# ruffle-rs/h263-rs

Hardware: NVIDIA B200
Metric: decoded_rgba_megapixels_per_s (higher is better)
Workload: dtype f32+u8

## Files before the change

### h263_rs_b200/csrc/context.cu

```cuda
#include <cuda_runtime.h>

#include <algorithm>
#include <chrono>
#include <cstdio>
#include <cstdlib>
#include <cstring>
#include <mutex>
#include <new>
#include <vector>

#include "device_math.cuh"
#include "kernels.cuh"

using namespace h263dev;

namespace h263fe {
int parse_step_deferred(h263cu_parser* const* parsers, const uint8_t* const* packets, const size_t* lens,
                        const uint32_t* stream_ids, uint32_t n, int threads, h263cu_pic* pics, h263cu_mb* mbs, uint32_t mb_cap,
                        h263cu_event* events, uint32_t ev_cap, uint32_t* n_pics_out, uint32_t* n_mbs_out, uint32_t* n_units_out,
                        int* per_pic_err, int32_t* pic_of_input, uint32_t max_w, uint32_t max_h);
void parse_step_finish(h263cu_parser* const* parsers, uint32_t n, bool accept);
}

extern "C" const uint8_t h263cu_quant_to_strength[32] = H263_QUANT_TO_STRENGTH;

namespace {

#define CU_TRY(expr)                      \
    do {                                  \
        cudaError_t _e = (expr);          \
        if (_e != cudaSuccess) return map_cuda_error(_e); \
    } while (0)

int map_cuda_error(cudaError_t e) {
    switch (e) {
        case cudaErrorNoDevice:
        case cudaErrorInsufficientDriver:
        case cudaErrorInvalidDevice: return H263CU_ERR_NO_DEVICE;
        case cudaErrorMemoryAllocation: return H263CU_ERR_OUT_OF_MEMORY;
        default: return H263CU_ERR_CUDA;
    }
}

inline size_t round_up(size_t v, size_t a) { return (v + a - 1) / a * a; }

struct StreamState {
    bool has_pic = false;
    uint8_t cur_slot = 0;
    int8_t rgba_slot = -1;
    uint16_t w = 0, h = 0;
    uint8_t pic_type = 0, pquant = 0;
    uint16_t tr = 0;
    uint32_t stamp = 0;
    uint32_t seen = 0;
    bool has_ref = false;
    uint8_t ref_slot = 0;
    uint16_t ref_w = 0, ref_h = 0;
    bool padded = false;
};

inline int next_slot(const StreamState& st) { return st.has_ref ? (st.ref_slot ^ 1) : (st.has_pic ? (st.cur_slot ^ 1) : 0); }

inline void advance_stream(StreamState& st, const h263cu_pic& p, bool want_rgba, int rgba_ring, bool tiled) {
    const int slot = next_slot(st);
    st.cur_slot = (uint8_t)slot;
    st.has_pic = true;
    st.w = p.width, st.h = p.height;
    st.pic_type = p.pic_type, st.pquant = p.pquant, st.tr = p.temporal_reference;
    st.rgba_slot = want_rgba ? (int8_t)rgba_ring : (int8_t)-1;
    if (!(p.flags & H263CU_PICFLAG_DISPOSABLE)) {
        st.has_ref = true;
        st.ref_slot = (uint8_t)slot;
        st.ref_w = p.width, st.ref_h = p.height;
        st.padded = tiled;
    }
}

}

struct h263cu_step {
    std::vector<h263cu_pic> pics;
    h263cu_mb* d_mbs = nullptr;
    h263cu_event* d_events = nullptr;
    uint32_t n_mbs = 0, n_units = 0;
    size_t mb_cap = 0, ev_cap = 0;
    uint32_t max_w = 0, max_h = 0;
};

struct h263cu_ctx {
    int device = 0;
    uint32_t max_streams = 0, max_w = 0, max_h = 0;
    uint32_t mbw = 0, mbh = 0;
    uint32_t pitch_y = 0, pitch_c = 0, rgba_pitch = 0;
    size_t y_slot = 0, c_slot = 0, rgba_slot = 0;
    uint8_t *y_pool = nullptr, *c_pool = nullptr, *rgba_pool = nullptr;
    CUtensorMap rgba_map;
    std::vector<StreamState> streams;
    uint32_t stamp = 0, decode_epoch = 0;
    uint32_t rgba_parity = 0;

    cudaStream_t s_main = nullptr, s_h2d = nullptr, s_d2h = nullptr;
    cudaStream_t s_pics = nullptr;
    static constexpr int PIC_RING = 4;
    PicDev* h_pics[PIC_RING] = {};
    PicDev* d_pics[PIC_RING] = {};
    cudaEvent_t pics_done[PIC_RING] = {};
    cudaEvent_t pics_up[PIC_RING] = {};
    size_t pics_cap = 0;
    int pic_ring_pos = 0;
    h263cu_step ring[2];
    cudaEvent_t ring_h2d_done[2] = {}, ring_run_done[2] = {};
    int ring_pos = 0;
    struct Staging {
        h263cu_pic* pics = nullptr;
        h263cu_mb* mbs = nullptr;
        h263cu_event* events = nullptr;
        size_t pic_cap = 0, mb_cap = 0, ev_cap = 0;
    } staging[2];
    std::vector<int32_t> pic_of_input;
    std::vector<uint64_t> rgba_offsets;
    cudaEvent_t rgba_written[2] = {}, rgba_read[2] = {};
    cudaEvent_t t0 = nullptr, t1 = nullptr;
    uint64_t launches = 0, tiled_launches = 0;
    bool profiling = false;
    std::vector<cudaEvent_t> prof_free;
    struct ProfSpan {
        cudaEvent_t a, b;
        int kind;
    };
    std::vector<ProfSpan> prof_spans;
    ChecksumJob* d_jobs = nullptr;
    unsigned long long* d_sums = nullptr;
    size_t jobs_cap = 0;

    int force_kernel = 0;
    double host_parse_s = 0.0, host_other_s = 0.0;
    uint64_t host_calls = 0;
    uint8_t* plane(int p, uint32_t stream, int slot) const {
        const size_t idx = (size_t)stream * 2 + (size_t)slot;
        if (p == 0) return y_pool + idx * y_slot + (size_t)PAD_Y_ROWS * pitch_y + PAD_Y_COLS;
        return c_pool + idx * c_slot + (size_t)PAD_C_ROWS * pitch_c + PAD_C_COLS + (p == 2 ? 1 : 0);
    }
    uint8_t* rgba(uint32_t stream, int slot) const { return rgba_pool + ((size_t)slot * max_streams + stream) * rgba_slot; }
};

namespace {

int ensure_pic_ring(h263cu_ctx* c, size_t n) {
    if (n <= c->pics_cap) return 0;
    CU_TRY(cudaStreamSynchronize(c->s_main));
    size_t cap = std::max<size_t>(n, 256);
    for (int i = 0; i < h263cu_ctx::PIC_RING; i++) {
        if (c->h_pics[i]) cudaFreeHost(c->h_pics[i]);
        if (c->d_pics[i]) cudaFree(c->d_pics[i]);
        c->h_pics[i] = nullptr, c->d_pics[i] = nullptr;
        CU_TRY(cudaHostAlloc((void**)&c->h_pics[i], cap * sizeof(PicDev), cudaHostAllocDefault));
        CU_TRY(cudaMalloc((void**)&c->d_pics[i], cap * sizeof(PicDev)));
    }
    c->pics_cap = cap;
    return 0;
}

int step_reserve(h263cu_step* s, size_t n_mbs, size_t n_units) {
    if (n_mbs > s->mb_cap) {
        if (s->d_mbs) cudaFree(s->d_mbs);
        s->d_mbs = nullptr;
        size_t cap = n_mbs + n_mbs / 8 + 64;
        CU_TRY(cudaMalloc((void**)&s->d_mbs, cap * sizeof(h263cu_mb)));
        s->mb_cap = cap;
    }
    if (n_units + 8 > s->ev_cap) {
        if (s->d_events) cudaFree(s->d_events);
        s->d_events = nullptr;
        size_t cap = n_units + n_units / 8 + 64;
        CU_TRY(cudaMalloc((void**)&s->d_events, cap * sizeof(h263cu_event)));
        s->ev_cap = cap;
    }
    return 0;
}

int prof_take(h263cu_ctx* c, cudaEvent_t* a, cudaEvent_t* b) {
    for (cudaEvent_t* e : {a, b}) {
        if (!c->prof_free.empty()) {
            *e = c->prof_free.back();
            c->prof_free.pop_back();
        } else {
            CU_TRY(cudaEventCreate(e));
        }
    }
    return 0;
// ... 3 lines not shown
    c->prof_spans.push_back({a, b, kind});
}

PicDev make_picdev(const h263cu_ctx* c, const h263cu_pic& p, const StreamState& st, bool want_rgba, int rgba_ring) {
    const int ref_slot = st.ref_slot, new_slot = next_slot(st);
    PicDev d;
    std::memset(&d, 0, sizeof(d));
    for (int k = 0; k < 3; k++) {
        d.cur[k] = c->plane(k, p.stream, new_slot);
        d.ref[k] = st.has_ref ? c->plane(k, p.stream, ref_slot) : nullptr;
    }
    d.rgba = want_rgba ? c->rgba(p.stream, rgba_ring) : nullptr;
    d.cur_y4 = (uint32_t)((d.cur[0] - c->y_pool) >> 2);
    d.cur_c4 = (uint32_t)((d.cur[1] - c->c_pool) >> 2);
    d.ref_y4 = st.has_ref ? (uint32_t)((d.ref[0] - c->y_pool) >> 2) : 0u;
    d.ref_c4 = st.has_ref ? (uint32_t)((d.ref[1] - c->c_pool) >> 2) : 0u;
    d.rgba_row0 = want_rgba ? (uint32_t)((size_t)(d.rgba - c->rgba_pool) / c->rgba_pitch) : 0u;
    d.first_event = p.first_event;
    d.rgba_pitch = c->rgba_pitch;
    d.w = p.width, d.h = p.height;
    d.cw = (uint16_t)((p.width + 1) / 2), d.ch = (uint16_t)((p.height + 1) / 2);
    d.pitch_y = (uint16_t)c->pitch_y, d.pitch_c = (uint16_t)c->pitch_c;
    d.strength = h263cu_quant_to_strength[p.pquant & 31];
    d.flags = p.flags;
    return d;
}

int run_step(h263cu_ctx* c, h263cu_step* s, uint32_t out_flags, bool lean = false) {
    const uint32_t n = (uint32_t)s->pics.size();
    if (n == 0) return 0;
    if (n > 65535) return H263CU_ERR_CAPACITY;
    const bool want_rgba = (out_flags & H263CU_OUT_RGBA) != 0;
    const bool want_deblock = want_rgba && (out_flags & H263CU_OUT_DEBLOCK) != 0;
    const uint32_t stamp = ++c->stamp;
    uint32_t max_w = 0, max_h = 0;
    bool tiled = true, aligned16 = true, wide_mv = false;
    for (uint32_t i = 0; i < n; i++) {
        const h263cu_pic& p = s->pics[i];
        if (p.stream >= c->max_streams) return H263CU_ERR_CAPACITY;
        if (p.width == 0 || p.height == 0 || p.width > c->max_w || p.height > c->max_h) return H263CU_ERR_CAPACITY;
        if ((uint32_t)p.mb_w * 16 < p.width || (uint32_t)p.mb_h * 16 < p.height ||
            (uint32_t)p.mb_w > c->mbw || (uint32_t)p.mb_h > c->mbh)
            return H263CU_ERR_BAD_ARGUMENT;
        if ((uint64_t)p.first_mb + p.n_mbs > s->n_mbs || (uint64_t)p.first_event + p.n_event_units > s->n_units ||
            p.n_mbs != (uint32_t)p.mb_w * p.mb_h)
            return H263CU_ERR_BAD_ARGUMENT;
        StreamState& st = c->streams[p.stream];
        if (st.stamp == stamp) return H263CU_ERR_BAD_ARGUMENT;
        st.stamp = stamp;
        if (p.flags & H263CU_PICFLAG_HAS_INTER) {
            if (!st.has_ref) return H263CU_ERR_UNCODED_IFRAME_BLOCKS;
            if (st.ref_w != p.width || st.ref_h != p.height) return H263CU_ERR_REFERENCE_WOULD_ABORT;
        }
        max_w = std::max<uint32_t>(max_w, p.width);
        max_h = std::max<uint32_t>(max_h, p.height);
        if ((p.width | p.height) & 15) aligned16 = false;
        if ((p.flags & H263CU_PICFLAG_HAS_INTER) && !(p.flags & H263CU_PICFLAG_MV_IN_RANGE)) wide_mv = true;
        if ((p.flags & H263CU_PICFLAG_HAS_INTER) && !st.padded) tiled = false;
    }
    if (c->force_kernel == 1) tiled = false;
    int e = ensure_pic_ring(c, n);
    if (e) return e;
    const int slot = c->pic_ring_pos;
    CU_TRY(cudaEventSynchronize(c->pics_done[slot]));
    const int rgba_ring = (int)(c->rgba_parity & 1u);
    PicDev* hp = c->h_pics[slot];
    for (uint32_t i = 0; i < n; i++) {
        const h263cu_pic& p = s->pics[i];
        const PicDev d = make_picdev(c, p, c->streams[p.stream], want_rgba, rgba_ring);
        hp[i] = d;
    }
    cudaEvent_t pa = nullptr, pb = nullptr, qa = nullptr, qb = nullptr;
    if (c->profiling) {
        if ((e = prof_take(c, &pa, &pb))) return e;
        if (want_deblock && (e = prof_take(c, &qa, &qb))) {
            c->prof_free.push_back(pa), c->prof_free.push_back(pb);
            return e;
        }
    }
    if (lean) {
        CU_TRY(cudaMemcpyAsync(c->d_pics[slot], hp, n * sizeof(PicDev), cudaMemcpyHostToDevice, c->s_main));
    } else {
        CU_TRY(cudaMemcpyAsync(c->d_pics[slot], hp, n * sizeof(PicDev), cudaMemcpyHostToDevice, c->s_pics));
        CU_TRY(cudaEventRecord(c->pics_up[slot], c->s_pics));
        CU_TRY(cudaStreamWaitEvent(c->s_main, c->pics_up[slot], 0));
    }
    if (want_rgba) {
        CU_TRY(cudaStreamWaitEvent(c->s_main, c->rgba_read[rgba_ring], 0));
    }
    if (pa) cudaEventRecord(pa, c->s_main);
    const Pools pools{c->y_pool, c->c_pool, c->rgba_pool, c->pitch_y, c->pitch_c, c->rgba_pitch};
    launch_recon(c->d_pics[slot], s->d_mbs, s->d_events, s->n_mbs, want_rgba && !want_deblock, tiled ? (aligned16 ? 1 : 2) : 0, wide_mv, pools,
                 &c->rgba_map, c->s_main);
    if (pa) prof_end(c, pa, pb, 0);
    if (want_deblock) {
        if (qa) cudaEventRecord(qa, c->s_main);
        if (aligned16 && c->force_kernel != 1)
            launch_deblock_rgba_tile(c->d_pics[slot], n, max_w, max_h, c->s_main);
        else
            launch_deblock_rgba(c->d_pics[slot], n, max_w, max_h, c->s_main);
        if (qa) prof_end(c, qa, qb, 1);
    }
    CU_TRY(cudaGetLastError());
    c->pic_ring_pos = (c->pic_ring_pos + 1) % h263cu_ctx::PIC_RING;
    c->launches += want_deblock ? 2 : 1;
    if (tiled) c->tiled_launches++;
    for (uint32_t i = 0; i < n; i++) advance_stream(c->streams[s->pics[i].stream], s->pics[i], want_rgba, rgba_ring, tiled);
    CU_TRY(cudaEventRecord(c->pics_done[slot], c->s_main));
    if (want_rgba) {
        if (!lean) CU_TRY(cudaEventRecord(c->rgba_written[rgba_ring], c->s_main));
        c->rgba_parity++;
    }
    return 0;
}

int validate_side_info(std::vector<h263cu_pic>& pics, const h263cu_mb* mbs, uint32_t n_mbs, uint32_t n_units) {
    for (size_t i = 0; i < pics.size(); i++) {
        h263cu_pic& p = pics[i];
        if ((uint64_t)p.first_mb + p.n_mbs > n_mbs || (uint64_t)p.first_event + p.n_event_units > n_units ||
            p.n_mbs != (uint32_t)p.mb_w * p.mb_h || p.mb_w == 0)
            return H263CU_ERR_BAD_ARGUMENT;
        bool any_inter = false, in_range = true;
        const h263cu_mb* m = mbs + p.first_mb;
        for (uint32_t k = 0; k < p.n_mbs; k++, m++) {
            if (m->pic != i || (uint32_t)m->mby * p.mb_w + m->mbx != k || m->mbx >= p.mb_w) return H263CU_ERR_BAD_ARGUMENT;
            uint32_t ev = 0;
            for (int b = 0; b < 6; b++) ev += m->nev[b];
            if (m->flags & H263CU_MB_WIDE) ev *= 2;
            if ((uint64_t)m->ev_off + ev > p.n_event_units) return H263CU_ERR_BAD_ARGUMENT;
            if (m->flags & H263CU_MB_INTER) {
                any_inter = true;
                for (int b = 0; b < 4; b++)
                    in_range &= m->u.mv[b][0] >= -32 && m->u.mv[b][0] <= 31 && m->u.mv[b][1] >= -32 && m->u.mv[b][1] <= 31;
            }
        }
        if (any_inter) p.flags |= H263CU_PICFLAG_HAS_INTER;
        if (!in_range) p.flags &= (uint8_t)~H263CU_PICFLAG_MV_IN_RANGE;
    }
    return 0;
}

int upload_into(h263cu_ctx* c, h263cu_step* s, const h263cu_pic* pics, uint32_t n_pics, const h263cu_mb* mbs,
                uint32_t n_mbs, const h263cu_event* events, uint32_t n_units, cudaStream_t stream, bool trusted) {
    int e = step_reserve(s, n_mbs, n_units);
    if (e) return e;
    try {
        s->pics.assign(pics, pics + n_pics);
    } catch (const std::bad_alloc&) {
        return H263CU_ERR_OUT_OF_MEMORY;
    }
    s->n_mbs = n_mbs, s->n_units = n_units;
    if (!trusted && (e = validate_side_info(s->pics, mbs, n_mbs, n_units))) {
        s->pics.clear();
        return e;
    }
    if (n_mbs) CU_TRY(cudaMemcpyAsync(s->d_mbs, mbs, (size_t)n_mbs * sizeof(h263cu_mb), cudaMemcpyHostToDevice, stream));
    if (n_units)
        CU_TRY(cudaMemcpyAsync(s->d_events, events, (size_t)n_units * sizeof(h263cu_event), cudaMemcpyHostToDevice, stream));
    (void)c;
    return 0;
}

template <typename T>
int grow_pinned(T** p, size_t* cap, size_t need) {
    if (need <= *cap) return 0;
    if (*p) cudaFreeHost(*p);
    *p = nullptr, *cap = 0;
    const size_t n = need + need / 4 + 64;
    CU_TRY(cudaHostAlloc((void**)p, n * sizeof(T), cudaHostAllocDefault));
    *cap = n;
    return 0;
// ... 17 lines not shown
        return H263CU_ERR_CUDA;
    return 0;
}
void free_step_buffers(h263cu_step* s) {
    if (s->d_mbs) cudaFree(s->d_mbs);
    if (s->d_events) cudaFree(s->d_events);
    s->d_mbs = nullptr, s->d_events = nullptr;
    s->mb_cap = s->ev_cap = 0;
}

}

extern "C" {

int h263cu_device_count(void) {
    int n = 0;
    if (cudaGetDeviceCount(&n) != cudaSuccess) {
        cudaGetLastError();
        return 0;
    }
    return n;
}

h263cu_ctx* h263cu_create(int device, uint32_t max_streams, uint32_t max_width, uint32_t max_height, uint32_t flags,
                          int* err) {
    (void)flags;
    int dummy;
    if (!err) err = &dummy;
    *err = 0;
    if (max_streams == 0 || max_width == 0 || max_height == 0 || max_width > 4080 || max_height > 4080) {
        *err = H263CU_ERR_BAD_ARGUMENT;
        return nullptr;
    }
    int ndev = 0;
    cudaError_t ce = cudaGetDeviceCount(&ndev);
    if (ce != cudaSuccess || ndev == 0) {
        cudaGetLastError();
        *err = H263CU_ERR_NO_DEVICE;
        return nullptr;
    }
    if (device < 0 || device >= ndev) {
        *err = H263CU_ERR_NO_DEVICE;
        return nullptr;
    }
    if (cudaSetDevice(device) != cudaSuccess) {
        *err = H263CU_ERR_CUDA;
        return nullptr;
    }
    h263cu_ctx* c = new (std::nothrow) h263cu_ctx();
    if (!c) {
        *err = H263CU_ERR_OUT_OF_MEMORY;
        return nullptr;
    }
    c->device = device;
    c->max_streams = max_streams, c->max_w = max_width, c->max_h = max_height;
    c->mbw = (max_width + 15) / 16, c->mbh = (max_height + 15) / 16;
    c->pitch_y = c->mbw * 16 + 2 * PAD_Y_COLS;
    c->pitch_c = c->mbw * 8 * CHROMA_STEP + 2 * PAD_C_COLS;
    c->rgba_pitch = c->mbw * 16 * 4;
    c->y_slot = (size_t)c->pitch_y * (c->mbh * 16 + 2 * PAD_Y_ROWS);
    c->c_slot = (size_t)c->pitch_c * (c->mbh * 8 + 2 * PAD_C_ROWS);
    if (const char* k = getenv("H263CU_KERNEL")) c->force_kernel = !strcmp(k, "mb") ? 1 : (!strcmp(k, "tile") ? 2 : 0);
    c->rgba_slot = (size_t)c->rgba_pitch * c->mbh * 16;
    c->streams.resize(max_streams);
    auto fail = [&](int code) {
        *err = code;
        h263cu_destroy(c);
        return (h263cu_ctx*)nullptr;
    };
    const size_t pad = 256;
    if (c->y_slot * 2 * max_streams + pad >= (16ull << 30) || c->rgba_slot * 2 * max_streams + pad >= (64ull << 30)) return fail(H263CU_ERR_CAPACITY);
    if (cudaMalloc((void**)&c->y_pool, c->y_slot * 2 * max_streams + pad) != cudaSuccess) return fail(H263CU_ERR_OUT_OF_MEMORY);
    if (cudaMalloc((void**)&c->c_pool, c->c_slot * 2 * max_streams + pad) != cudaSuccess) return fail(H263CU_ERR_OUT_OF_MEMORY);
    if (cudaMalloc((void**)&c->rgba_pool, c->rgba_slot * 2 * max_streams + pad) != cudaSuccess) return fail(H263CU_ERR_OUT_OF_MEMORY);
    {
        const int e = make_rgba_map(&c->rgba_map, c->rgba_pool, c->rgba_pitch, (uint64_t)2 * max_streams * c->mbh * 16);
        if (e) return fail(e);
    }
    if (cudaStreamCreateWithFlags(&c->s_main, cudaStreamNonBlocking) != cudaSuccess) return fail(H263CU_ERR_CUDA);
    if (cudaStreamCreateWithFlags(&c->s_h2d, cudaStreamNonBlocking) != cudaSuccess) return fail(H263CU_ERR_CUDA);
    if (cudaStreamCreateWithFlags(&c->s_d2h, cudaStreamNonBlocking) != cudaSuccess) return fail(H263CU_ERR_CUDA);
    if (cudaStreamCreateWithFlags(&c->s_pics, cudaStreamNonBlocking) != cudaSuccess) return fail(H263CU_ERR_CUDA);
    for (int i = 0; i < h263cu_ctx::PIC_RING; i++)
        if (cudaEventCreateWithFlags(&c->pics_done[i], cudaEventDisableTiming) != cudaSuccess ||
            cudaEventCreateWithFlags(&c->pics_up[i], cudaEventDisableTiming) != cudaSuccess)
            return fail(H263CU_ERR_CUDA);
    for (int i = 0; i < 2; i++) {
        if (cudaEventCreateWithFlags(&c->ring_h2d_done[i], cudaEventDisableTiming) != cudaSuccess ||
            cudaEventCreateWithFlags(&c->ring_run_done[i], cudaEventDisableTiming) != cudaSuccess ||
            cudaEventCreateWithFlags(&c->rgba_written[i], cudaEventDisableTiming) != cudaSuccess ||
            cudaEventCreateWithFlags(&c->rgba_read[i], cudaEventDisableTiming) != cudaSuccess)
            return fail(H263CU_ERR_CUDA);
    }
    if (cudaEventCreate(&c->t0) != cudaSuccess || cudaEventCreate(&c->t1) != cudaSuccess) return fail(H263CU_ERR_CUDA);
    cudaMemsetAsync(c->y_pool, 0, c->y_slot * 2 * max_streams + pad, c->s_main);
    cudaMemsetAsync(c->c_pool, 0, c->c_slot * 2 * max_streams + pad, c->s_main);
    if (cudaStreamSynchronize(c->s_main) != cudaSuccess) return fail(H263CU_ERR_CUDA);
    return c;
}

void h263cu_destroy(h263cu_ctx* c) {
    if (!c) return;
    cudaSetDevice(c->device);
    if (c->s_main) cudaStreamSynchronize(c->s_main);
    if (c->s_h2d) cudaStreamSynchronize(c->s_h2d);
    if (c->s_d2h) cudaStreamSynchronize(c->s_d2h);
    if (c->s_pics) cudaStreamSynchronize(c->s_pics);
    for (int i = 0; i < 2; i++) free_step_buffers(&c->ring[i]);
    for (auto& st : c->staging) {
        if (st.pics) cudaFreeHost(st.pics);
        if (st.mbs) cudaFreeHost(st.mbs);
        if (st.events) cudaFreeHost(st.events);
    }
    for (int i = 0; i < h263cu_ctx::PIC_RING; i++) {
        if (c->h_pics[i]) cudaFreeHost(c->h_pics[i]);
        if (c->d_pics[i]) cudaFree(c->d_pics[i]);
        if (c->pics_done[i]) cudaEventDestroy(c->pics_done[i]);
        if (c->pics_up[i]) cudaEventDestroy(c->pics_up[i]);
    }
    for (int i = 0; i < 2; i++) {
        if (c->ring_h2d_done[i]) cudaEventDestroy(c->ring_h2d_done[i]);
        if (c->ring_run_done[i]) cudaEventDestroy(c->ring_run_done[i]);
        if (c->rgba_written[i]) cudaEventDestroy(c->rgba_written[i]);
        if (c->rgba_read[i]) cudaEventDestroy(c->rgba_read[i]);
    }
    if (c->t0) cudaEventDestroy(c->t0);
    if (c->t1) cudaEventDestroy(c->t1);
    for (auto& sp : c->prof_spans) {
        cudaEventDestroy(sp.a);
        cudaEventDestroy(sp.b);
    }
    for (auto e : c->prof_free) cudaEventDestroy(e);
    if (c->d_jobs) cudaFree(c->d_jobs);
    if (c->d_sums) cudaFree(c->d_sums);
    if (c->y_pool) cudaFree(c->y_pool);
    if (c->c_pool) cudaFree(c->c_pool);
    if (c->rgba_pool) cudaFree(c->rgba_pool);
    if (c->s_main) cudaStreamDestroy(c->s_main);
    if (c->s_h2d) cudaStreamDestroy(c->s_h2d);
    if (c->s_d2h) cudaStreamDestroy(c->s_d2h);
    if (c->s_pics) cudaStreamDestroy(c->s_pics);
    delete c;
}

int h263cu_device_of(h263cu_ctx* c) { return c ? c->device : -1; }

void* h263cu_alloc_pinned(size_t bytes) {
    void* p = nullptr;
    if (cudaHostAlloc(&p, bytes ? bytes : 1, cudaHostAllocDefault) != cudaSuccess) {
        cudaGetLastError();
        return nullptr;
    }
    return p;
}
void h263cu_free_pinned(void* p) {
    if (p) cudaFreeHost(p);
}

h263cu_step* h263cu_step_upload(h263cu_ctx* c, const h263cu_pic* pics, uint32_t n_pics, const h263cu_mb* mbs,
                                uint32_t n_mbs, const h263cu_event* events, uint32_t n_units, int* err) {
    int dummy;
    if (!err) err = &dummy;
    *err = 0;
    if (!c || !pics || (!mbs && n_mbs) || (!events && n_units)) {
        *err = H263CU_ERR_BAD_ARGUMENT;
        return nullptr;
    }
    cudaSetDevice(c->device);
    h263cu_step* s = new (std::nothrow) h263cu_step();
    if (!s) {
        *err = H263CU_ERR_OUT_OF_MEMORY;
        return nullptr;
    }
    int e = upload_into(c, s, pics, n_pics, mbs, n_mbs, events, n_units, c->s_main, false);
    if (e) {
        free_step_buffers(s);
        delete s;
        *err = e;
        return nullptr;
    }
    return s;
}

void h263cu_step_free(h263cu_ctx* c, h263cu_step* s) {
    if (!s) return;
    if (c) {
        cudaSetDevice(c->device);
        cudaStreamSynchronize(c->s_main);
    }
    free_step_buffers(s);
    delete s;
}

int h263cu_step_run(h263cu_ctx* c, h263cu_step* s, uint32_t out_flags) {
    if (!c || !s) return H263CU_ERR_BAD_ARGUMENT;
    cudaSetDevice(c->device);
    return run_step(c, s, out_flags);
}

static int submit_common(h263cu_ctx* c, const h263cu_pic* pics, uint32_t n_pics, const h263cu_mb* mbs, uint32_t n_mbs,
                         const h263cu_event* events, uint32_t n_units, uint32_t out_flags, bool trusted = false, bool lean = false) {
// ... 653 lines not shown
```

### h263_rs_b200/csrc/recon_tile.cu

```cuda
#include "recon_common.cuh"

namespace h263dev {

namespace {

constexpr int WARP_MBS = 4;
#ifndef H263_STD_WARPS
#define H263_STD_WARPS 5
#endif
#ifndef H263_STD_CTAS
#define H263_STD_CTAS 7
#endif
constexpr int GEN_WARPS = 4, GEN_CTAS = 8;
#ifndef H263_ABLATE
#define H263_ABLATE 0
#endif
#ifndef H263_RGBA_TMA
#define H263_RGBA_TMA 1
#endif
#ifndef H263_RGBA_MODE
#define H263_RGBA_MODE 4
#endif
constexpr int WARP_BLOCKS = WARP_MBS * 6;
constexpr int RES_WORDS = 36;
constexpr int EV_CAP = 64;
constexpr int SLOT_FLOATS = 68;
constexpr int STAGE_BYTES = 4096;

constexpr uint32_t MBF_INTER = 1u << 0;
constexpr uint32_t MBF_LEFT = 1u << 2, MBF_RIGHT = 1u << 3, MBF_TOP = 1u << 4, MBF_BOTTOM = 1u << 5;
constexpr uint32_t MBF_RGBA = 1u << 6;
constexpr uint32_t BF_SLOW = 1u << 4;

struct __align__(16) WarpStage {
    uint32_t res[WARP_BLOCKS][RES_WORDS];
    uint32_t evbuf[EV_CAP];
    uint2 slotdesc[WARP_BLOCKS];
    uint32_t sstart[WARP_BLOCKS];
    uint32_t slotinfo[WARP_BLOCKS];
};
static_assert(sizeof(WarpStage) == STAGE_BYTES, "the RGBA tile aliases exactly this");

template <bool COMPACT>
struct WarpTailT;
template <>
struct __align__(16) WarpTailT<true> {
    float coef[4][SLOT_FLOATS];
    uint4 mba[WARP_MBS];
    uint32_t bd[WARP_BLOCKS];
    uint32_t meta[WARP_BLOCKS];
    uint8_t bf[WARP_BLOCKS];
    __device__ __forceinline__ uint32_t* mbrec() { return reinterpret_cast<uint32_t*>(&coef[0][0]); }
};
template <>
struct __align__(16) WarpTailT<false> {
    float coef[4][SLOT_FLOATS];
    uint4 mba[WARP_MBS];
    uint4 mbb[WARP_MBS];
    uint32_t bd[WARP_BLOCKS];
    uint32_t meta[WARP_BLOCKS];
    uint32_t mbrec_[WARP_BLOCKS];
    uint8_t bf[WARP_BLOCKS];
    __device__ __forceinline__ uint32_t* mbrec() { return mbrec_; }
};

template <bool COMPACT, int NW>
struct TileSmemT {
    WarpStage stage[NW];
    WarpTailT<COMPACT> tail[NW];
};
static_assert(sizeof(TileSmemT<true, H263_STD_WARPS>) <= 200704 / H263_STD_CTAS - 1024, "shared memory budget of the standard instantiations");
static_assert(sizeof(TileSmemT<false, GEN_WARPS>) <= 200704 / GEN_CTAS - 1024, "shared memory budget of the generic instantiations");

__device__ const float g_basis[8][8] = H263_BASIS_TABLE;
__device__ const uint8_t g_dezigzag[64] = H263_DEZIGZAG_LINEAR;

__device__ __forceinline__ constexpr float k_basis(int y, int j) {
    constexpr float T[8][8] = H263_BASIS_TABLE;
    return T[y][j];
}

__device__ __forceinline__ int dequant_narrow(int level, int q2, int qc) {
    const int mag = q2 * abs(level) + qc;
    const int v = level < 0 ? -mag : mag;
    return max(min(v, 2047), -2048);
}

__device__ __forceinline__ int round_q(float q, float m) { return __float2int_rz(fadd(fmul(q, m), copysign_half(q))); }

struct RowSum {
    uint32_t lo, hi;
};
__device__ __forceinline__ RowSum row_sum4(uint32_t w0, uint32_t w1, int sh, int shb) {
    const uint32_t a = __funnelshift_r(w0, w1, sh), b = __funnelshift_rc(w0, w1, shb);
    RowSum h;
    h.hi = __byte_perm(a, 0, 0x4341) + __byte_perm(b, 0, 0x4341);
    h.lo = (a + b) - 256u * h.hi;
    return h;
}
__device__ __forceinline__ uint32_t vmix(uint32_t top, uint32_t bottom, uint32_t wt, uint32_t wb) {
    return __byte_perm(top * wt + (bottom * wb + 0x00800080u), 0, 0x4341);
}

#if H263_RGBA_MODE == 0 || H263_RGBA_MODE == 3
__device__ __forceinline__ uint32_t pack_sat(int a, int b, uint32_t c) {
    uint32_t d;
    asm("cvt.pack.sat.u8.s32.b32 %0, %1, %2, %3;" : "=r"(d) : "r"(a), "r"(b), "r"(c));
    return d;
}
#endif
struct CT {
    int r, g, b;
};
__device__ __forceinline__ int opaque(int v) {
    asm("" : "+r"(v));
    return v;
}
#if H263_RGBA_MODE == 0 || H263_RGBA_MODE == 3
__device__ __forceinline__ CT chroma_terms_folded(int cb, int cr, int kr, int kg, int kb) {
    CT t;
    t.r = cr * kr + (32768 - 128 * 104597 - 16 * 76309);
    t.g = cr * kg + (cb * -25675 + (32768 + 128 * 53279 + 128 * 25675 - 16 * 76309));
    t.b = cb * kb + (32768 - 128 * 132201 - 16 * 76309);
    return t;
}
#else
__device__ __forceinline__ CT chroma_terms_folded(int cb, int cr, int kr, int kg, int kb) {
    CT t;
    t.r = cr * kr + (0xFFFFFF - (32768 - 128 * 104597 - 16 * 76309));
    t.g = cr * kg + (cb * 25675 + (0xFFFFFF - (32768 + 128 * 53279 + 128 * 25675 - 16 * 76309)));
    t.b = cb * kb + (0xFFFFFF - (32768 - 128 * 132201 - 16 * 76309));
#if H263_RGBA_MODE == 4
    t.g = cr * (kg - kr) + (cb * 25675 + ((32768 - 128 * 104597) - (32768 + 128 * 53279 + 128 * 25675)));
    t.b = cb * kb + (cr * -kr + ((32768 - 128 * 104597) - (32768 - 128 * 132201)));
#endif
    return t;
}
#endif
#if H263_RGBA_MODE == 0
__device__ __forceinline__ uint32_t rgba_px(uint32_t yw, int k, int ky, const CT& t) {
    const int y = (int)(__byte_perm(yw, 0, 0x4440 + k));
    const int r = (y * ky + t.r) >> 16, g = (y * ky + t.g) >> 16, b = (y * ky + t.b) >> 16;
    return pack_sat(g, r, pack_sat(255, b, 0));
}
#elif H263_RGBA_MODE == 3
__device__ __forceinline__ uint32_t rgba_px(uint32_t yw, int k, int ky, const CT& t) {
    const int y = (int)__dp4a(yw, 1u << (8 * k), 0u);
    const int r = __dp2a_hi(y * ky + t.r, 0x01000000, 0), g = __dp2a_hi(y * ky + t.g, 0x01000000, 0), b = __dp2a_hi(y * ky + t.b, 0x01000000, 0);
    return pack_sat(g, r, pack_sat(255, b, 0));
}
#else
__device__ __forceinline__ uint32_t rgba_px(uint32_t yw, int k, int ky, const CT& t) {
#if H263_RGBA_MODE == 1
    const int y = (int)(__byte_perm(yw, 0, 0x4440 + k));
#else
    const int y = (int)__dp4a(yw, 1u << (8 * k), 0u);
#endif
#if H263_RGBA_MODE == 4
    const int xr = y * ky + t.r;
    const uint32_t wr = (uint32_t)__vimin_s32_relu(xr, 0xFFFFFF), wg = (uint32_t)__viaddmin_s32_relu(xr, t.g, 0xFFFFFF),
                   wb = (uint32_t)__viaddmin_s32_relu(xr, t.b, 0xFFFFFF);
#else
    const int nyk = opaque(y * ky);
    const uint32_t wr = (uint32_t)__viaddmin_s32_relu(nyk, t.r, 0xFFFFFF), wg = (uint32_t)__viaddmin_s32_relu(nyk, t.g, 0xFFFFFF),
                   wb = (uint32_t)__viaddmin_s32_relu(nyk, t.b, 0xFFFFFF);
#endif
    const uint32_t rg = __byte_perm(wr, wg, 0x3362);
    uint32_t px;
    asm("lop3.b32 %0, %1, %2, 0xFFFF0000, 0x07;" : "=r"(px) : "r"(rg), "r"(wb));
    return px;
}
#endif

__device__ __forceinline__ uint32_t scan_up_step(uint32_t v, int d) {
    asm volatile("{ .reg .pred p; .reg .b32 t; shfl.sync.up.b32 t|p, %0, %1, 0, 0xffffffff; @p add.u32 %0, %0, t; }" : "+r"(v) : "r"(d));
    return v;
}
__device__ __forceinline__ int seg_scan_up_step(int v, int d, int dist) {
    asm volatile("{ .reg .pred p; .reg .b32 t; shfl.sync.up.b32 t, %0, %1, 0, 0xffffffff; setp.ge.s32 p, %2, %1; @p add.s32 %0, %0, t; }"
                 : "+r"(v)
                 : "r"(d), "r"(dist));
    return v;
}

__device__ __forceinline__ uint32_t mad_pack(uint32_t o, uint32_t e) { return o * 256u + e; }

__device__ __forceinline__ uint32_t merge_bytes(uint32_t a, uint32_t b, int keep) {
    const uint32_t m = keep >= 4 ? 0xFFFFFFFFu : ((1u << (8 * keep)) - 1u);
    return (a & m) | (b & ~m);
}

__device__ __forceinline__ uint32_t stage_offset(int q, int row, int c) { return (uint32_t)(q * 1024 + row * 64 + c * 16); }

}


template <int PY, int PC, int PR, bool EDGE, bool WIDE_MV, int NW, int NCTAS>
__global__ void __launch_bounds__(NW * 32, NCTAS)
    recon_tile_kernel(const PicDev* __restrict__ pics, const h263cu_mb* __restrict__ mbs,
                      const h263cu_event* __restrict__ events, uint32_t n_mbs, int emit_rgba, const Pools pools,
                      const __grid_constant__ CUtensorMap rgba_map) {
    constexpr bool COMPACT = PY != 0 && !EDGE && !WIDE_MV;
    constexpr int CTA_WARPS = NW;
    __shared__ __align__(1024) TileSmemT<COMPACT, NW> S;
    const int tid = threadIdx.x, lane = tid & 31, warp = tid >> 5;
    WarpStage& G = S.stage[warp];
    WarpTailT<COMPACT>& W = S.tail[warp];
    uint32_t* const mbrec = W.mbrec();
    const int g = lane >> 3, t = lane & 7;
    const uint32_t lt_mask = (1u << lane) - 1u;

    const uint32_t n_tiles = (n_mbs + WARP_MBS - 1) / WARP_MBS;
    const uint32_t tile = blockIdx.x * CTA_WARPS + warp;
    if (tile >= n_tiles) return;
    const uint32_t mb0 = tile * WARP_MBS;
    const int n_w = (int)min((uint32_t)WARP_MBS, n_mbs - mb0);

    if (lane < n_w * 6) mbrec[lane] = __ldg(reinterpret_cast<const uint32_t*>(mbs) + (size_t)tile * WARP_BLOCKS + lane);
    __syncwarp();
    int n_slots;
    {
        const bool bvalid = lane < n_w * 6;
        const int bm = bvalid ? (lane * 43) >> 8 : 0, bb = bvalid ? lane - bm * 6 : 0;
        const uint32_t* r = &mbrec[bm * 6];
        const uint32_t w0 = r[0], w1 = r[1], w2 = r[2], w3 = r[3], w4 = r[4], w5 = r[5];
        const uint32_t pic = w1 & 0xFFFFu;
        const PicDev& P = pics[pic];
        const int mbx = (w1 >> 16) & 0xFF, mby = w1 >> 24;
        const bool inter = (w2 & H263CU_MB_INTER) != 0, wide = (w2 & H263CU_MB_WIDE) != 0;
        const uint32_t nev = bvalid ? __byte_perm(w2, w3, 0x4440u + (uint32_t)bb + 2u) & 0xFFu : 0u;
        const uint32_t code = inter ? 0u : __byte_perm(w4, w5, 0x4440u + (uint32_t)bb) & 0xFFu;

        uint32_t boff = 0, bflags = 0;
        if (inter) {
            int mvx, mvy, bx, sy, pitch;
            uint32_t base;
            bool in_range;
            if (bb < 4) {
                const int m = (int)((bb < 2 ? w4 : w5) >> (16 * (bb & 1)));
                mvx = __dp4a(m, 0x00000001, 0), mvy = __dp4a(m, 0x00000100, 0);
                in_range = mvx >= -32 && mvx <= 31 && mvy >= -32 && mvy <= 31;
                bx = mbx * 16 + (bb & 1) * 8 + (mvx >> 1), sy = mby * 16 + (bb >> 1) * 8 + (mvy >> 1);
                pitch = PY ? PY : P.pitch_y, base = P.ref_y4;
            } else {
                const int sx = __dp4a((int)w5, 0x00010001, __dp4a((int)w4, 0x00010001, 13));
                const int sy13 = __dp4a((int)w5, 0x01000100, __dp4a((int)w4, 0x01000100, 13));
                mvx = (sx >> 4) + ((sx - 11) >> 4), mvy = (sy13 >> 4) + ((sy13 - 11) >> 4);
                in_range = mvx >= -16 && mvx <= 15 && mvy >= -16 && mvy <= 15;
                bx = 2 * (mbx * 8 + (mvx >> 1)), sy = mby * 8 + (mvy >> 1);
                pitch = PC ? PC : P.pitch_c, base = P.ref_c4;
            }
            const int a = bx & 3;
            boff = base + (uint32_t)((sy * pitch + (bx - a)) >> 2);
            bflags = (uint32_t)(a | ((mvx & 1) << 2) | ((mvy & 1) << 3)) | (!WIDE_MV || in_range ? 0u : BF_SLOW);
        }
        if (bvalid) {
            W.bd[lane] = boff;
            W.bf[lane] = (uint8_t)bflags;
            if (bb == 0) {
                const int pitch_y = PY ? PY : P.pitch_y, pitch_c = PC ? PC : P.pitch_c;
                const int mbw = (P.w + 15) >> 4, mbh = (P.h + 15) >> 4;
                const uint32_t ed = EDGE ? ((uint32_t)(P.w & 15) | ((uint32_t)(P.h & 15) << 4) | ((uint32_t)(P.cw & 7) << 8) |
                                            ((uint32_t)(P.ch & 7) << 12))
                                         : 0u;
                uint32_t flags = inter ? MBF_INTER : 0u;
                if (mbx == 0) flags |= MBF_LEFT;
                if (mbx == mbw - 1) flags |= MBF_RIGHT;
                if (mby == 0) flags |= MBF_TOP;
                if (mby == mbh - 1) flags |= MBF_BOTTOM;
                if (emit_rgba && P.rgba) flags |= MBF_RGBA;
                W.mba[bm] = make_uint4(P.cur_y4 + (uint32_t)((mby * 16 * pitch_y + mbx * 16) >> 2),
                                       P.cur_c4 + (uint32_t)((mby * 8 * pitch_c + mbx * 16) >> 2), P.rgba_row0 + (uint32_t)(mby * 16),
                                       flags | ((uint32_t)mbx << 8));
                if constexpr (!COMPACT) W.mbb[bm] = make_uint4((uint32_t)pitch_y | ((uint32_t)pitch_c << 16), 0u, pic, ed);
            }
        }

        const bool coded = nev > 0;
        const uint32_t coded_mask = __ballot_sync(FULL, coded);
        const int pos = __popc(coded_mask & lt_mask);
        n_slots = __popc(coded_mask);
        uint32_t ev_incl = nev;
#pragma unroll
        for (int d = 1; d < 32; d <<= 1) ev_incl = scan_up_step(ev_incl, d);
        const uint32_t before = (ev_incl - nev) - __shfl_sync(FULL, ev_incl - nev, bm * 6);
        if (coded) {
            G.sstart[pos] = ev_incl - nev;
            const uint32_t first = P.first_event + w0 + (wide ? 2 * before : before);
            const uint32_t quant = (w2 >> 8) & 31u;
            G.slotdesc[pos] = make_uint2(first, nev | (quant << 8) | (wide ? 1u << 13 : 0u) | (inter ? 1u << 14 : 0u) |
                                                    (bb >= 4 ? 1u << 15 : 0u) | ((uint32_t)lane << 16) | (code << 24));
            asm volatile("prefetch.global.L1 [%0];" ::"l"(events + first));
        } else if (bvalid) {
            const bool has_dc = code != 0;
            const int dcres = has_dc ? round_residual_dc((float)intradc_level((int)code)) : 0;
            W.meta[lane] = (uint32_t)(has_dc ? CLS_DC : CLS_ZERO) | ((uint32_t)dcres << 16);
        }
// ... 98 lines not shown
                     ((my_sd.y & 0xFFu) << 22) | ((my_sd.y & 0x8000u) << 15);
                const int n = __popc(R);
                key = n >= 4 ? 0 : (n >= 2 ? 1 : (n == 1 ? 2 : 3));
            }
            int pos = s_lo, n_need = 0;
#pragma unroll
            for (int j = 0; j < 3; j++) {
                const uint32_t b = __ballot_sync(FULL, key == j);
                if (j < key) pos += __popc(b);
                if (j == key) pos += __popc(b & lt_mask);
                n_need += __popc(b);
            }
            __syncwarp();
            if (key < 3) G.slotinfo[pos] = pd;
            __syncwarp();

            for (int si0 = s_lo; si0 < s_lo + n_need; si0 += 4) {
                const int si = si0 + g;
                const bool valid = si < s_lo + n_need;
                const uint32_t pd = valid ? G.slotinfo[si] : 0u;
                const int sl = (int)(pd & 31u);
                const uint32_t R = (pd >> 5) & 0xFFu;
                const bool vert = (pd >> 13) & 1u;
                const int nev = (int)((pd >> 22) & 0xFFu);
                const uint32_t first = (pd >> 15) & 127u;
                *reinterpret_cast<float4*>(c + t * 8) = make_float4(0.f, 0.f, 0.f, 0.f);
                *reinterpret_cast<float4*>(c + t * 8 + 4) = make_float4(0.f, 0.f, 0.f, 0.f);
                const int nevmax = __reduce_max_sync(FULL, nev);
                __syncwarp();
                if (t < nev) {
                    const uint32_t ent = G.evbuf[first + t];
                    c[ent & 63u] = (float)((int)ent >> 16);
                }
                if (nevmax > 8) {
                    for (int k = t + 8; k < nev; k += 8) {
                        const uint32_t ent = G.evbuf[first + k];
                        c[ent & 63u] = (float)((int)ent >> 16);
                    }
                }
                if (pd & 0x4000u) {
                    if (t == 0) c[0] = (float)intradc_level((int)(G.slotdesc[sl].y >> 24));
                }
                const uint32_t U = __reduce_or_sync(FULL, R);
                __syncwarp();
                float acc[8] = {0.f, 0.f, 0.f, 0.f, 0.f, 0.f, 0.f, 0.f};
#pragma unroll
                for (int y = 0; y < 8; y++) {
                    if (!((U >> y) & 1u)) continue;
                    const float4 ca = *reinterpret_cast<const float4*>(c + y * 8);
                    const float4 cc = *reinterpret_cast<const float4*>(c + y * 8 + 4);
                    float a = fmul(ca.x, bt0);
                    a = fadd(a, fmul(ca.y, bt1));
                    a = fadd(a, fmul(ca.z, bt2));
                    a = fadd(a, fmul(ca.w, bt3));
                    a = fadd(a, fmul(cc.x, bt4));
                    a = fadd(a, fmul(cc.y, bt5));
                    a = fadd(a, fmul(cc.z, bt6));
                    a = fadd(a, fmul(cc.w, bt7));
                    if (vert) a = ca.x;
                    a = fmul(a, 0.25f);
#pragma unroll
                    for (int j = 0; j < 8; j++) acc[j] = fadd(acc[j], fmul(a, k_basis(y, j)));
                }
                const bool any_vert = __any_sync(FULL, vert);
                if (R) {
                    uint16_t* rrow = reinterpret_cast<uint16_t*>(&G.res[sl][0]) + ((pd & 0x40000000u) ? t : tperm);
                    if (any_vert) {
                        const float m = vert ? H263_B00 : 1.0f;
#pragma unroll
                        for (int j = 0; j < 8; j++) rrow[j * 8] = (uint16_t)(int16_t)round_q(acc[j], m);
                    } else {
#pragma unroll
                        for (int j = 0; j < 8; j++) rrow[j * 8] = (uint16_t)(int16_t)__float2int_rz(fadd(acc[j], copysign_half(acc[j])));
                    }
                }
                __syncwarp();
            }
            s_lo = s_hi;
            e_lo = e_end;
        }
    }

    {
        const int mbq = lane >> 3, rgrp = (lane >> 2) & 1, cg = lane & 3;
        const bool unit_ok = mbq < n_w;
        const int mbi = unit_ok ? mbq : 0;
        const uint4 ma = W.mba[mbi];
        uint4 mv = make_uint4(0u, (ma.w >> 8) & 0xFFu, 0u, 0u);
        if constexpr (!COMPACT) {
            const uint4 b = W.mbb[mbi];
            mv.x = b.x, mv.z = b.z, mv.w = b.w;
        }
        const uint32_t flags = (unit_ok ? ma.w : 0u) & ~((H263_ABLATE & 2) ? MBF_INTER : 0u) & ~((H263_ABLATE & 4) ? MBF_RGBA : 0u);
        const uint32_t pitch_y4 = PY ? PY / 4 : (mv.x & 0xFFFFu) >> 2, pitch_c4 = PC ? PC / 4 : mv.x >> 18;
        const int lb = rgrp * 2 + (cg >> 1);
        const int bl = mbi * 6 + lb, bc = mbi * 6 + 4;

        uint32_t ylo[8], yhi[8];
        uint32_t cbp[4], crp[4];
        if (flags & MBF_INTER) {
            const uint32_t fl = W.bf[bl], fc = W.bf[bc];
            if (!WIDE_MV || !(fl & BF_SLOW)) {
                const int sh = (fl & 3u) * 8, shb = sh + ((fl & 4u) << 1);
                const uint32_t wb = ((fl >> 3) & 1u) * 64u, wt = 128u - wb;
                const bool second = (fl & 7u) != 0;
                const uint32_t* src = reinterpret_cast<const uint32_t*>(pools.y) + W.bd[bl] + (uint32_t)(cg & 1);
                RowSum hs[9];
#pragma unroll
                for (int r = 0; r < 9; r++) {
                    const uint32_t* p = src + (uint32_t)r * pitch_y4;
                    uint32_t w0 = 0u, w1 = 0u;
                    if (r < 8 || wb != 0) {
                        w0 = __ldg(p);
                        if (second) w1 = __ldg(p + 1);
                    }
                    hs[r] = row_sum4(w0, w1, sh, shb);
                }
#pragma unroll
                for (int r = 0; r < 8; r++) {
                    ylo[r] = vmix(hs[r].lo, hs[r + 1].lo, wt, wb);
                    yhi[r] = vmix(hs[r].hi, hs[r + 1].hi, wt, wb);
                }
            } else {
                const PicDev& P = pics[mv.z];
                const uint32_t* rr = &mbrec[mbi * 6];
                const uint32_t w1 = rr[1];
                const uint32_t mvw = lb < 2 ? (rr[4] >> (16 * lb)) : (rr[5] >> (16 * (lb - 2)));
                const int mvx = (int8_t)(mvw & 0xFF), mvy = (int8_t)((mvw >> 8) & 0xFF);
                const int x0 = (int)((w1 >> 16) & 0xFF) * 16 + cg * 4, y0 = (int)(w1 >> 24) * 16 + rgrp * 8;
#pragma unroll
                for (int r = 0; r < 8; r++) {
                    uint32_t s[4];
#pragma unroll
                    for (int k = 0; k < 4; k++) s[k] = mc_fetch1(P.ref[0], P.pitch_y, 1, P.w, P.h, x0 + k, y0 + r, mvx, mvy);
                    ylo[r] = s[0] | (s[2] << 16), yhi[r] = s[1] | (s[3] << 16);
                }
            }
            if (!WIDE_MV || !(fc & BF_SLOW)) {
                const int sh = (fc & 3u) * 8, shb = sh + ((fc & 4u) << 2);
                const uint32_t wb = ((fc >> 3) & 1u) * 64u, wt = 128u - wb;
                const bool second = (fc & 7u) != 0;
                const uint32_t* src = reinterpret_cast<const uint32_t*>(pools.c) + W.bd[bc] + (uint32_t)cg + (uint32_t)(rgrp * 4) * pitch_c4;
                RowSum hs[5];
#pragma unroll
                for (int r = 0; r < 5; r++) {
                    const uint32_t* p = src + (uint32_t)r * pitch_c4;
                    uint32_t w0 = 0u, w1 = 0u;
                    if (r < 4 || wb != 0) {
                        w0 = __ldg(p);
                        if (second) w1 = __ldg(p + 1);
                    }
                    hs[r] = row_sum4(w0, w1, sh, shb);
                }
#pragma unroll
                for (int r = 0; r < 4; r++) {
                    cbp[r] = vmix(hs[r].lo, hs[r + 1].lo, wt, wb);
                    crp[r] = vmix(hs[r].hi, hs[r + 1].hi, wt, wb);
                }
            } else {
                const PicDev& P = pics[mv.z];
                const uint32_t* rr = &mbrec[mbi * 6];
                const uint32_t w1 = rr[1], w4 = rr[4], w5 = rr[5];
                const int sumx = (int8_t)byte_of(w4, 0) + (int8_t)byte_of(w4, 2) + (int8_t)byte_of(w5, 0) + (int8_t)byte_of(w5, 2);
                const int sumy = (int8_t)byte_of(w4, 1) + (int8_t)byte_of(w4, 3) + (int8_t)byte_of(w5, 1) + (int8_t)byte_of(w5, 3);
                const int mvx = average_sum_of_mvs(sumx), mvy = average_sum_of_mvs(sumy);
                const int x0 = (int)((w1 >> 16) & 0xFF) * 8 + cg * 2, y0 = (int)(w1 >> 24) * 8 + rgrp * 4;
// ... 132 lines not shown
                    uint4 px;
                    px.x = rgba_px(yw[r], 0, ky, t0);
                    px.y = rgba_px(yw[r], 1, ky, t0);
                    px.z = rgba_px(yw[r], 2, ky, t1);
                    px.w = rgba_px(yw[r], 3, ky, t1);
#if H263_RGBA_TMA
                    *reinterpret_cast<uint4*>(stage + stage_offset(mbq, rgrp * 8 + r, cg)) = px;
#else
                    if (H263_ABLATE & 16) {
                        if ((px.x ^ px.y ^ px.z ^ px.w) == 0x12345678u) *reinterpret_cast<uint4*>(o + (size_t)r * rgba_pitch) = px;
                    } else
                        *reinterpret_cast<uint4*>(o + (size_t)r * rgba_pitch) = px;
#endif
                }
            }
        }
#if H263_RGBA_TMA
        asm volatile("fence.proxy.async.shared::cta;" ::: "memory");
        __syncwarp();
        if (lane < n_w) {
            const uint32_t f = W.mba[lane].w & ~((H263_ABLATE & (4 | 16)) ? MBF_RGBA : 0u);
            if (f & MBF_RGBA) {
                const uint32_t src = (uint32_t)__cvta_generic_to_shared(&G) + (uint32_t)lane * 1024u;
                asm volatile("cp.async.bulk.tensor.2d.global.shared::cta.bulk_group [%0, {%2, %3}], [%1];" ::"l"(&rgba_map), "r"(src),
                             "r"((int)((f >> 8 & 0xFFu) * 64u)), "r"((int)W.mba[lane].z)
                             : "memory");
                asm volatile("cp.async.bulk.commit_group;" ::: "memory");
            }
        }
#endif

        if (unit_ok && !(H263_ABLATE & 8)) {
            const uint32_t pitch_y = pitch_y4 * 4, pitch_c = pitch_c4 * 4;
            uint8_t* py = pools.y + (size_t)(ma.x + (uint32_t)(rgrp * 8) * pitch_y4 + (uint32_t)cg) * 4;
            uint8_t* pc = pools.c + (size_t)(ma.y + (uint32_t)(rgrp * 4) * pitch_c4 + (uint32_t)cg) * 4;
#pragma unroll
            for (int r = 0; r < 8; r++) *reinterpret_cast<uint32_t*>(py + r * pitch_y) = yw[r];
#pragma unroll
            for (int r = 0; r < 4; r++) *reinterpret_cast<uint32_t*>(pc + r * pitch_c) = cw[r];
            const bool e_left = (flags & MBF_LEFT) && cg == 0, e_right = (flags & MBF_RIGHT) && cg == 3;
            const bool e_top = (flags & MBF_TOP) && rgrp == 0, e_bot = (flags & MBF_BOTTOM) && rgrp == 1;
            if (e_left | e_right | e_top | e_bot) {
                const ptrdiff_t side = e_left ? -16 : 4;
                if (e_left | e_right) {
#pragma unroll
                    for (int r = 0; r < 8; r++) {
                        const uint32_t v = __byte_perm(yw[r], 0, e_left ? 0x0000 : 0x3333);
                        *reinterpret_cast<uint4*>(py + r * pitch_y + side) = make_uint4(v, v, v, v);
                    }
#pragma unroll
                    for (int r = 0; r < 4; r++) {
                        const uint32_t v = __byte_perm(cw[r], 0, e_left ? 0x1010 : 0x3232);
                        *reinterpret_cast<uint4*>(pc + r * pitch_c + side) = make_uint4(v, v, v, v);
                    }
                }
                if (e_top | e_bot) {
                    const bool corner = e_left | e_right;
                    const uint32_t v = e_top ? yw[0] : yw[7];
                    uint8_t* rowp = e_top ? py : py + 7 * pitch_y;
                    const ptrdiff_t dir = e_top ? -(ptrdiff_t)pitch_y : (ptrdiff_t)pitch_y;
                    const uint32_t vc = __byte_perm(v, 0, e_left ? 0x0000 : 0x3333);
                    for (int k = 1; k <= 16; k++) {
                        uint8_t* d = rowp + k * dir;
                        *reinterpret_cast<uint32_t*>(d) = v;
                        if (corner) *reinterpret_cast<uint4*>(d + side) = make_uint4(vc, vc, vc, vc);
                    }
                    const uint32_t c = e_top ? cw[0] : cw[3];
                    uint8_t* rc = e_top ? pc : pc + 3 * pitch_c;
                    const ptrdiff_t cdir = e_top ? -(ptrdiff_t)pitch_c : (ptrdiff_t)pitch_c;
                    const uint32_t cc = __byte_perm(c, 0, e_left ? 0x1010 : 0x3232);
                    for (int k = 1; k <= 8; k++) {
                        uint8_t* d = rc + k * cdir;
                        *reinterpret_cast<uint32_t*>(d) = c;
                        if (corner) *reinterpret_cast<uint4*>(d + side) = make_uint4(cc, cc, cc, cc);
                    }
                }
            }
        }

#if H263_RGBA_TMA
        asm volatile("cp.async.bulk.wait_group.read 0;" ::: "memory");
#endif
    }
}

int recon_tile_uses_tma() { return H263_RGBA_TMA; }

void launch_recon_tile(const PicDev* pics, const h263cu_mb* mbs, const h263cu_event* events, uint32_t n_mbs, int emit_rgba,
                       int unaligned, int wide_mv, const Pools& pools, const CUtensorMap* rgba_map, cudaStream_t stream) {
    if (n_mbs == 0) return;
    const uint32_t py = pools.pitch_y, pc = pools.pitch_c, pr = pools.rgba_pitch;
    const CUtensorMap& tm = *rgba_map;
#define H263_LAUNCH(PY_, PC_, PR_, EDGE_, WIDE_, NW_, NCTAS_)                                                                      \
    recon_tile_kernel<PY_, PC_, PR_, EDGE_, WIDE_, NW_, NCTAS_>                                                                    \
        <<<(n_mbs + NW_ * WARP_MBS - 1) / (NW_ * WARP_MBS), NW_ * 32, 0, stream>>>(pics, mbs, events, n_mbs, emit_rgba, pools, tm)
    if (wide_mv) {
        if (unaligned)
            H263_LAUNCH(0, 0, 0, true, true, GEN_WARPS, GEN_CTAS);
        else
            H263_LAUNCH(0, 0, 0, false, true, GEN_WARPS, GEN_CTAS);
    } else if (unaligned)
        H263_LAUNCH(0, 0, 0, true, false, GEN_WARPS, GEN_CTAS);
    else if (py == 416 && pc == 416 && pr == 1408)
        H263_LAUNCH(416, 416, 1408, false, false, H263_STD_WARPS, H263_STD_CTAS);
    else if (py == 240 && pc == 240 && pr == 704)
        H263_LAUNCH(240, 240, 704, false, false, H263_STD_WARPS, H263_STD_CTAS);
    else if (py == 768 && pc == 768 && pr == 2816)
        H263_LAUNCH(768, 768, 2816, false, false, H263_STD_WARPS, H263_STD_CTAS);
    else
        H263_LAUNCH(0, 0, 0, false, false, GEN_WARPS, GEN_CTAS);
#undef H263_LAUNCH
}

}
```

Measured before the change: 467,900.

## Use programmatic dependent launch for recon tile and host-sync pic upload

Launches the tiled reconstruction kernel with programmatic stream serialization, so each CTA triggers dependents early and waits on the prior grid only before its output stage, overlapping its prologue with the previous kernel. The picture-descriptor upload on the side stream is now followed by a host cudaStreamSynchronize instead of an event wait, and the rgba-read wait is skipped when the event has already completed. It also adds an optional CTA timing trace compiled out by default. The host synchronize blocks the CPU on every step, and the early griddepcontrol placement may weaken ordering for work that reads earlier outputs before the wait.

```diff
diff --git a/h263_rs_b200/csrc/context.cu b/h263_rs_b200/csrc/context.cu
--- a/h263_rs_b200/csrc/context.cu
+++ b/h263_rs_b200/csrc/context.cu
@@ -105,7 +105,6 @@
     PicDev* h_pics[PIC_RING] = {};
     PicDev* d_pics[PIC_RING] = {};
     cudaEvent_t pics_done[PIC_RING] = {};
-    cudaEvent_t pics_up[PIC_RING] = {};
     size_t pics_cap = 0;
     int pic_ring_pos = 0;
     h263cu_step ring[2];
@@ -275,11 +274,14 @@
         CU_TRY(cudaMemcpyAsync(c->d_pics[slot], hp, n * sizeof(PicDev), cudaMemcpyHostToDevice, c->s_main));
     } else {
         CU_TRY(cudaMemcpyAsync(c->d_pics[slot], hp, n * sizeof(PicDev), cudaMemcpyHostToDevice, c->s_pics));
-        CU_TRY(cudaEventRecord(c->pics_up[slot], c->s_pics));
-        CU_TRY(cudaStreamWaitEvent(c->s_main, c->pics_up[slot], 0));
+        CU_TRY(cudaStreamSynchronize(c->s_pics));
     }
     if (want_rgba) {
-        CU_TRY(cudaStreamWaitEvent(c->s_main, c->rgba_read[rgba_ring], 0));
+        const cudaError_t q = cudaEventQuery(c->rgba_read[rgba_ring]);
+        if (q == cudaErrorNotReady)
+            CU_TRY(cudaStreamWaitEvent(c->s_main, c->rgba_read[rgba_ring], 0));
+        else if (q != cudaSuccess)
+            return map_cuda_error(q);
     }
     if (pa) cudaEventRecord(pa, c->s_main);
     const Pools pools{c->y_pool, c->c_pool, c->rgba_pool, c->pitch_y, c->pitch_c, c->rgba_pitch};
@@ -463,9 +465,7 @@
     if (cudaStreamCreateWithFlags(&c->s_d2h, cudaStreamNonBlocking) != cudaSuccess) return fail(H263CU_ERR_CUDA);
     if (cudaStreamCreateWithFlags(&c->s_pics, cudaStreamNonBlocking) != cudaSuccess) return fail(H263CU_ERR_CUDA);
     for (int i = 0; i < h263cu_ctx::PIC_RING; i++)
-        if (cudaEventCreateWithFlags(&c->pics_done[i], cudaEventDisableTiming) != cudaSuccess ||
-            cudaEventCreateWithFlags(&c->pics_up[i], cudaEventDisableTiming) != cudaSuccess)
-            return fail(H263CU_ERR_CUDA);
+        if (cudaEventCreateWithFlags(&c->pics_done[i], cudaEventDisableTiming) != cudaSuccess) return fail(H263CU_ERR_CUDA);
     for (int i = 0; i < 2; i++) {
         if (cudaEventCreateWithFlags(&c->ring_h2d_done[i], cudaEventDisableTiming) != cudaSuccess ||
             cudaEventCreateWithFlags(&c->ring_run_done[i], cudaEventDisableTiming) != cudaSuccess ||
@@ -497,7 +497,6 @@
         if (c->h_pics[i]) cudaFreeHost(c->h_pics[i]);
         if (c->d_pics[i]) cudaFree(c->d_pics[i]);
         if (c->pics_done[i]) cudaEventDestroy(c->pics_done[i]);
-        if (c->pics_up[i]) cudaEventDestroy(c->pics_up[i]);
     }
     for (int i = 0; i < 2; i++) {
         if (c->ring_h2d_done[i]) cudaEventDestroy(c->ring_h2d_done[i]);
diff --git a/h263_rs_b200/csrc/recon_tile.cu b/h263_rs_b200/csrc/recon_tile.cu
--- a/h263_rs_b200/csrc/recon_tile.cu
+++ b/h263_rs_b200/csrc/recon_tile.cu
@@ -75,6 +75,24 @@
 __device__ const float g_basis[8][8] = H263_BASIS_TABLE;
 __device__ const uint8_t g_dezigzag[64] = H263_DEZIGZAG_LINEAR;
 
+#ifndef H263_CTA_TRACE
+#define H263_CTA_TRACE 0
+#endif
+#if H263_CTA_TRACE
+constexpr uint32_t CTA_TRACE_CAP = 1u << 20;
+__device__ unsigned long long g_cta_trace[CTA_TRACE_CAP][4];
+__device__ uint32_t g_cta_trace_n;
+__device__ __forceinline__ unsigned long long global_timer() {
+    unsigned long long t;
+    asm volatile("mov.u64 %0, %%globaltimer;" : "=l"(t));
+    return t;
+}
+#define H263_TRACE_EXIT() \
+    if (lane == 0 && trace_i < CTA_TRACE_CAP) atomicMax(&g_cta_trace[trace_i][1], global_timer())
+#else
+#define H263_TRACE_EXIT()
+#endif
+
 __device__ __forceinline__ constexpr float k_basis(int y, int j) {
     constexpr float T[8][8] = H263_BASIS_TABLE;
     return T[y][j];
@@ -209,10 +227,30 @@
     uint32_t* const mbrec = W.mbrec();
     const int g = lane >> 3, t = lane & 7;
     const uint32_t lt_mask = (1u << lane) - 1u;
+#if H263_CTA_TRACE
+    __shared__ uint32_t trace_slot;
+    if (tid == 0) {
+        const uint32_t i = atomicAdd(&g_cta_trace_n, 1u);
+        trace_slot = i;
+        if (i < CTA_TRACE_CAP) {
+            uint32_t smid;
+            asm volatile("mov.u32 %0, %%smid;" : "=r"(smid));
+            g_cta_trace[i][0] = global_timer();
+            g_cta_trace[i][2] = smid | ((unsigned long long)blockIdx.x << 32);
+            g_cta_trace[i][3] = (unsigned long long)(uintptr_t)mbs;
+        }
+    }
+    __syncthreads();
+    const uint32_t trace_i = trace_slot;
+#endif
+    asm volatile("griddepcontrol.launch_dependents;" ::: "memory");
 
     const uint32_t n_tiles = (n_mbs + WARP_MBS - 1) / WARP_MBS;
     const uint32_t tile = blockIdx.x * CTA_WARPS + warp;
-    if (tile >= n_tiles) return;
+    if (tile >= n_tiles) {
+        H263_TRACE_EXIT();
+        return;
+    }
     const uint32_t mb0 = tile * WARP_MBS;
     const int n_w = (int)min((uint32_t)WARP_MBS, n_mbs - mb0);
 
@@ -477,6 +515,7 @@
     }
 
     {
+        asm volatile("griddepcontrol.wait;" ::: "memory");
         const int mbq = lane >> 3, rgrp = (lane >> 2) & 1, cg = lane & 3;
         const bool unit_ok = mbq < n_w;
         const int mbi = unit_ok ? mbq : 0;
@@ -775,6 +814,7 @@
         asm volatile("cp.async.bulk.wait_group.read 0;" ::: "memory");
 #endif
     }
+    H263_TRACE_EXIT();
 }
 
 int recon_tile_uses_tma() { return H263_RGBA_TMA; }
@@ -784,9 +824,21 @@
     if (n_mbs == 0) return;
     const uint32_t py = pools.pitch_y, pc = pools.pitch_c, pr = pools.rgba_pitch;
     const CUtensorMap& tm = *rgba_map;
+    cudaLaunchAttribute attr;
+    attr.id = cudaLaunchAttributeProgrammaticStreamSerialization;
+    attr.val.programmaticStreamSerializationAllowed = 1;
+    cudaLaunchConfig_t cfg = {};
+    cfg.dynamicSmemBytes = 0;
+    cfg.stream = stream;
+    cfg.attrs = &attr;
+    cfg.numAttrs = 1;
 #define H263_LAUNCH(PY_, PC_, PR_, EDGE_, WIDE_, NW_, NCTAS_)                                                                      \
-    recon_tile_kernel<PY_, PC_, PR_, EDGE_, WIDE_, NW_, NCTAS_>                                                                    \
-        <<<(n_mbs + NW_ * WARP_MBS - 1) / (NW_ * WARP_MBS), NW_ * 32, 0, stream>>>(pics, mbs, events, n_mbs, emit_rgba, pools, tm)
+    do {                                                                                                                           \
+        cfg.gridDim = dim3((n_mbs + NW_ * WARP_MBS - 1) / (NW_ * WARP_MBS));                                                       \
+        cfg.blockDim = dim3(NW_ * 32);                                                                                             \
+        cudaLaunchKernelEx(&cfg, recon_tile_kernel<PY_, PC_, PR_, EDGE_, WIDE_, NW_, NCTAS_>, pics, mbs, events, n_mbs, emit_rgba, \
+                           pools, tm);                                                                                             \
+    } while (0)
     if (wide_mv) {
         if (unaligned)
             H263_LAUNCH(0, 0, 0, true, true, GEN_WARPS, GEN_CTAS);
@@ -806,3 +858,19 @@
 }
 
 }
+
+#if H263_CTA_TRACE
+extern "C" int h263cu_cta_trace_read(unsigned long long* out, uint32_t cap, uint32_t* n) {
+    using namespace h263dev;
+    uint32_t cnt = 0;
+    if (cudaDeviceSynchronize() != cudaSuccess || cudaMemcpyFromSymbol(&cnt, g_cta_trace_n, sizeof(cnt)) != cudaSuccess) return -1;
+    const uint32_t m = cnt < cap ? (cnt < CTA_TRACE_CAP ? cnt : CTA_TRACE_CAP) : cap;
+    if (m && cudaMemcpyFromSymbol(out, g_cta_trace, (size_t)m * 4 * sizeof(unsigned long long)) != cudaSuccess) return -1;
+    void* p = nullptr;
+    if (cudaGetSymbolAddress(&p, g_cta_trace) != cudaSuccess || cudaMemset(p, 0, sizeof(g_cta_trace)) != cudaSuccess) return -1;
+    const uint32_t zero = 0;
+    if (cudaMemcpyToSymbol(g_cta_trace_n, &zero, sizeof(zero)) != cudaSuccess || cudaDeviceSynchronize() != cudaSuccess) return -1;
+    *n = cnt;
+    return 0;
+}
+#endif
```

Result: faster. 476,300 (median of 6 runs) (+1.8%).
